# 331658260/Drone-YOLO

Hardware: AMD Instinct MI355X
Metric: images/sec @640x640 Drone-YOLO-s (higher is better)
Workload: dtype fp16; 1 GPU; Drone-YOLO-s (yolov8s-p2-repvgg.yaml, nc=10) inference 640x640: layout+forward+decode+NMS, inputs resident in HBM; fp16 storage / fp32 accumulate (BASELINE config 2 names bf16: bf16 storage fails the IoU >= 0.999 bar - 0.995 - so the headline runs the 16-bit format that meets it; same MFMA rate, same bytes); batch_per_gpu=256, global_batch=256, parallelism=batch-split x1, no collective, hipgraph=True, streams=2, max_det=300

## Files before the change

drone-yolo_amd/csrc/layout_ops.hip:

```cpp
#include "common_hip.h"

namespace dy {

template <typename T>
__global__ __launch_bounds__(256) void nchw_to_nhwc_kernel(const float* __restrict__ src, T* __restrict__ dst, int n,
                                                           int c, int hw, int c_pad, int ld) {
  constexpr int EPC = Elem<T>::EPC;
  const long long total = (long long)n * hw;
  for (long long pix = (long long)blockIdx.x * 256 + threadIdx.x; pix < total; pix += (long long)gridDim.x * 256) {
    const int img = (int)(pix / hw);
    const int p = (int)(pix - (long long)img * hw);
    const float* s = src + (size_t)img * c * hw + p;
    T* d = dst + (size_t)pix * ld;
    for (int c0 = 0; c0 < c_pad; c0 += EPC) {
      float f[EPC];
#pragma unroll
      for (int e = 0; e < EPC; ++e) f[e] = (c0 + e < c) ? s[(size_t)(c0 + e) * hw] : 0.f;
      *reinterpret_cast<u32x4*>(d + c0) = Chunk<T>::pack(f);
    }
  }
}

__global__ __launch_bounds__(256) void nchw_to_nhwc_split_kernel(const float* __restrict__ src, unsigned char* __restrict__ dst, int n, int c, int hw, int c_pad, int ld) {
  const long long total = (long long)n * hw;
// ... 100 lines not shown
  u32x4* tmp = cur + tot;
  const int img = blockIdx.x / cgroups;
  const int cg = blockIdx.x - img * cgroups;
  const size_t base = (size_t)img * hw * ld + (size_t)cg * G * EPC;
  for (int i = threadIdx.x; i < tot; i += 512) {
    const int p = i / G, g = i - p * G;
    cur[i] = *reinterpret_cast<const u32x4*>(x + base + (size_t)p * ld + g * EPC);
  }
  __syncthreads();
  T* outs[3] = {y1, y2, y3};
#pragma unroll 1
  for (int pass = 0; pass < 3; ++pass) {
    for (int i = threadIdx.x; i < tot; i += 512) {
      const int p = i / G, g = i - p * G;
      const int yy = p / w, xx = p - yy * w;
      const int x0 = xx - r < 0 ? 0 : xx - r, x1 = xx + r >= w ? w - 1 : xx + r;
      u32x4 m = cur[(yy * w + x0) * G + g];
      for (int q = x0 + 1; q <= x1; ++q) m = chunk_max<T>(m, cur[(yy * w + q) * G + g]);
      tmp[i] = m;
    }
    __syncthreads();
    T* o = outs[pass];
    for (int i = threadIdx.x; i < tot; i += 512) {
      const int p = i / G, g = i - p * G;
      const int yy = p / w, xx = p - yy * w;
      const int y0 = yy - r < 0 ? 0 : yy - r, y1e = yy + r >= h ? h - 1 : yy + r;
      u32x4 m = tmp[(y0 * w + xx) * G + g];
      for (int q = y0 + 1; q <= y1e; ++q) m = chunk_max<T>(m, tmp[(q * w + xx) * G + g]);
      cur[i] = m;
      *reinterpret_cast<u32x4*>(o + base + (size_t)p * ld + g * EPC) = m;
    }
    __syncthreads();
  }
}

struct ChunkPair {
  u32x4 hi, lo;
};
__device__ __forceinline__ ChunkPair pair_max(const ChunkPair a, const ChunkPair b) {
  float fa[8], fb[8];
  join8(a.hi, a.lo, fa);
  join8(b.hi, b.lo, fb);
  const f16x8 ah = __builtin_bit_cast(f16x8, a.hi), al = __builtin_bit_cast(f16x8, a.lo), bh = __builtin_bit_cast(f16x8, b.hi), bl = __builtin_bit_cast(f16x8, b.lo);
  f16x8 h, l;
#pragma unroll
  for (int e = 0; e < 8; ++e) {
    const bool tb = fb[e] > fa[e];
    h[e] = tb ? bh[e] : ah[e];
    l[e] = tb ? bl[e] : al[e];
  }
  return ChunkPair{__builtin_bit_cast(u32x4, h), __builtin_bit_cast(u32x4, l)};
}

__global__ __launch_bounds__(512) void sppf_maxpool3_split_kernel(const unsigned char* __restrict__ x, unsigned char* __restrict__ y1, unsigned char* __restrict__ y2,
                                                                  unsigned char* __restrict__ y3, int h, int w, int cgroups, int G, int ld, int r) {
  extern __shared__ __attribute__((aligned(16))) unsigned char dyn_smem[];
  const int hw = h * w, tot = hw * G;
  ChunkPair* cur = reinterpret_cast<ChunkPair*>(dyn_smem);
  ChunkPair* tmp = cur + tot;
  const int img = blockIdx.x / cgroups;
  const int cg = blockIdx.x - img * cgroups;
  const size_t base = ((size_t)img * hw * ld + (size_t)cg * G * 8) * 4;
  for (int i = threadIdx.x; i < tot; i += 512) {
    const int p = i / G, g = i - p * G;
    const unsigned char* s = x + base + ((size_t)p * ld + g * 8) * 4;
    cur[i] = ChunkPair{*reinterpret_cast<const u32x4*>(s), *reinterpret_cast<const u32x4*>(s + 16)};
// ... 230 lines not shown
  const int epc = 16 / es;
  DY_REQUIRE(n > 0 && h > 0 && w > 0 && c > 0 && c % epc == 0 && ld >= c && ld % epc == 0, DY_ERR_INVALID_ARG,
             "dy_sppf_maxpool3: c/ld must be multiples of %d", epc);
  DY_REQUIRE(k >= 1 && (k & 1), DY_ERR_INVALID_ARG, "dy_sppf_maxpool3: k must be odd");
  DY_REQUIRE(aligned16(x) && aligned16(y1) && aligned16(y2) && aligned16(y3), DY_ERR_INVALID_ARG,
             "dy_sppf_maxpool3: views must be 16-byte aligned");
  DY_REQUIRE((long long)h * w <= 4608, DY_ERR_UNSUPPORTED, "dy_sppf_maxpool3: h*w=%d exceeds the LDS-resident limit 4608", h * w);
  hipStream_t st = reinterpret_cast<hipStream_t>(stream);
  const int cchunks = c / epc;
  int G = 1;
  for (int g = 8; g >= 1; --g)
    if (cchunks % g == 0 && (size_t)h * w * 32 * g <= 147456) {
      G = g;
      break;
    }
  const size_t smem = (size_t)h * w * 32 * G;
  const int cgroups = cchunks / G;
  if (dtype == DY_F16X2) {
    DY_REQUIRE(c % 8 == 0, DY_ERR_INVALID_ARG, "dy_sppf_maxpool3: DY_F16X2 needs c in groups of 8 channels");
    const int pairs = c / 8;
    int Gp = 1;
    for (int g = 4; g >= 1; --g)
      if (pairs % g == 0 && (size_t)h * w * 64 * g <= 147456) {
        Gp = g;
        break;
      }
    const size_t sm = (size_t)h * w * 64 * Gp;
    DY_REQUIRE(sm <= 147456, DY_ERR_UNSUPPORTED, "dy_sppf_maxpool3: DY_F16X2 map of %d pixels exceeds the LDS-resident limit", h * w);
    if (sm > 48 * 1024) (void)hipFuncSetAttribute((const void*)sppf_maxpool3_split_kernel, hipFuncAttributeMaxDynamicSharedMemorySize, (int)sm);
    hipLaunchKernelGGL(sppf_maxpool3_split_kernel, dim3((unsigned)(n * (pairs / Gp))), dim3(512), sm, st, (const unsigned char*)x, (unsigned char*)y1, (unsigned char*)y2,
                       (unsigned char*)y3, h, w, pairs / Gp, Gp, ld, k / 2);
    return check_launch("sppf_maxpool3_split_kernel");
  }
  const dim3 grid((unsigned)(n * cgroups));
#define DY_SPPF_LAUNCH(T)                                                                                          \
  do {                                                                                                              \
    if (smem > 48 * 1024)                                                                                           \
      (void)hipFuncSetAttribute((const void*)sppf_maxpool3_kernel<T>, hipFuncAttributeMaxDynamicSharedMemorySize,  \
                                (int)smem);                                                                         \
    hipLaunchKernelGGL((sppf_maxpool3_kernel<T>), grid, dim3(512), smem, st, (const T*)x, (T*)y1, (T*)y2, (T*)y3, h, \
                       w, cgroups, G, ld, k / 2);                                                                   \
  } while (0)
  if (dtype == DY_BF16)
    DY_SPPF_LAUNCH(bf16_t);
  else if (dtype == DY_F16)
    DY_SPPF_LAUNCH(f16_t);
  else if (dtype == DY_FP8)
    DY_SPPF_LAUNCH(fp8_t);
  else
    DY_SPPF_LAUNCH(float);
#undef DY_SPPF_LAUNCH
  return check_launch("sppf_maxpool3_kernel");
}

extern "C" int32_t dy_quantize_fp8_nhwc(const void* src, void* dst, int64_t rows, int32_t c, int32_t ld_src, int32_t ld_dst, int32_t src_dtype, float act_scale,
                                        dy_stream_t stream) {
  const int es = dtype_size_no_fp8(src_dtype);
  DY_REQUIRE(src && dst && es && rows > 0 && c > 0 && act_scale > 0.f, DY_ERR_INVALID_ARG, "dy_quantize_fp8_nhwc: bad arguments");
  DY_REQUIRE(c % 16 == 0 && ld_src >= c && ld_dst >= c && (ld_src * es) % 16 == 0 && ld_dst % 16 == 0 && aligned16(src) && aligned16(dst), DY_ERR_INVALID_ARG,
             "dy_quantize_fp8_nhwc: c must be a multiple of 16 and both views whole 16-byte chunks");
  hipStream_t st = reinterpret_cast<hipStream_t>(stream);
  const int grid = grid_for((long long)rows * (c / 16));
  const float inv = 1.f / act_scale;
  if (src_dtype == DY_BF16)
    hipLaunchKernelGGL((quantize_fp8_kernel<bf16_t>), dim3(grid), dim3(256), 0, st, (const bf16_t*)src, (fp8_t*)dst, (long long)rows, c / 16, ld_src, ld_dst, inv);
  else if (src_dtype == DY_F16)
    hipLaunchKernelGGL((quantize_fp8_kernel<f16_t>), dim3(grid), dim3(256), 0, st, (const f16_t*)src, (fp8_t*)dst, (long long)rows, c / 16, ld_src, ld_dst, inv);
  else
// ... 85 lines not shown
```

drone-yolo_amd/_lib.py:

```python
from __future__ import annotations

import ctypes as C
import os

_HERE = os.path.dirname(os.path.abspath(__file__))
LIB_PATH = os.path.join(_HERE, "lib", "libdyolo.so")

DY_BF16, DY_F16, DY_F32, DY_FP8, DY_F16X2 = 0, 1, 2, 3, 4
DY_ACT_NONE, DY_ACT_SILU, DY_ACT_SILU_L2E = 0, 1, 2
DY_MAX_LEVELS = 8
DY_WLAYOUT_ROWS, DY_WLAYOUT_HALO3X3, DY_WLAYOUT_FRAG1X1 = 0, 1, 2

_vp, _i32, _f32, _i64 = C.c_void_p, C.c_int32, C.c_float, C.c_int64


class PackJob(C.Structure):
    _fields_ = [("w", C.c_void_p), ("s_co", C.c_int64), ("s_ci", C.c_int64), ("s_r", C.c_int64), ("s_q", C.c_int64),
                ("cout", C.c_int32), ("cin", C.c_int32), ("ksize", C.c_int32), ("transpose_flip", C.c_int32), ("cin_logical", C.c_int32),
                ("w_layout", C.c_int32), ("dst", C.c_void_p), ("dst_elems", C.c_int64)]


class ConvDesc(C.Structure):

    _fields_ = [
# ... 92 lines not shown
        ("fuse_score", _i32), ("max_time_lost", _i32),
    ]


class LossDesc(C.Structure):

    _fields_ = [
        ("level", _vp * DY_MAX_LEVELS),
        ("h", _i32 * DY_MAX_LEVELS), ("w", _i32 * DY_MAX_LEVELS), ("ld", _i32 * DY_MAX_LEVELS),
        ("stride", _f32 * DY_MAX_LEVELS),
        ("n_levels", _i32), ("batch", _i32), ("nc", _i32), ("reg_max", _i32),
        ("gt", _vp), ("gmax", _i32), ("topk", _i32),
        ("alpha", _f32), ("beta", _f32), ("box_gain", _f32), ("cls_gain", _f32), ("dfl_gain", _f32),
        ("out", _vp), ("out_owner", _vp), ("workspace", _vp), ("workspace_bytes", _i64),
        ("grad_level", _vp * DY_MAX_LEVELS), ("ld_grad", _i32 * DY_MAX_LEVELS),
    ]


class C2fTailDesc(C.Structure):

    _fields_ = [
        ("t", _vp), ("buf", _vp), ("y", _vp), ("w3", _vp), ("b3", _vp), ("w1", _vp), ("b1", _vp),
        ("batch", _i32), ("h", _i32), ("w", _i32), ("hidden", _i32), ("cout", _i32), ("n_bottlenecks", _i32), ("shortcut", _i32),
        ("ld_t", _i32), ("ld_buf", _i32), ("ld_y", _i32), ("dtype", _i32), ("act_l2e", _i32),
    ]


class C2fFrontDesc(C.Structure):

    _fields_ = [
        ("x", _vp), ("other", _vp), ("y", _vp), ("w3", _vp), ("b3", _vp), ("w1", _vp), ("b1", _vp),
        ("batch", _i32), ("h", _i32), ("w", _i32), ("cin", _i32), ("cmid", _i32), ("c_other", _i32), ("cout", _i32),
        ("ld_x", _i32), ("ld_other", _i32), ("ld_y", _i32), ("act", _i32), ("dtype", _i32),
    ]


class C2fDesc(C.Structure):

    _fields_ = [
        ("x", _vp), ("x_lo", _vp), ("y", _vp), ("w_cv1", _vp), ("w_m_cv1", _vp), ("w_m_cv2", _vp), ("w_cv2", _vp), ("bias", _vp),
        ("batch", _i32), ("h", _i32), ("w", _i32), ("cin", _i32), ("cin_lo", _i32), ("hidden", _i32), ("cout", _i32),
        ("ld_x", _i32), ("ld_x_lo", _i32), ("ld_y", _i32), ("shortcut", _i32), ("dtype", _i32), ("act_l2e", _i32),
    ]


class Stem2Desc(C.Structure):

    _fields_ = [
        ("x", _vp), ("w0", _vp), ("b0", _vp), ("w1", _vp), ("b1", _vp), ("y", _vp),
        ("n", _i32), ("h", _i32), ("w", _i32), ("ld_y", _i32), ("act0", _i32), ("act1", _i32), ("dtype", _i32),
        ("w1_scale", _vp),
    ]


class BnDesc(C.Structure):

    _fields_ = [
        ("z", _vp), ("y", _vp), ("addend", _vp), ("dy", _vp), ("dz", _vp),
        ("rows", _i64),
        ("c", _i32), ("ld_z", _i32), ("ld_y", _i32), ("ld_add", _i32), ("ld_dy", _i32), ("ld_dz", _i32), ("dtype", _i32), ("act", _i32),
        ("gamma", _vp), ("beta", _vp), ("mean", _vp), ("rstd", _vp), ("running_mean", _vp), ("running_var", _vp),
        ("eps", _f32), ("momentum", _f32),
        ("dgamma", _vp), ("dbeta", _vp), ("workspace", _vp), ("workspace_bytes", _i64), ("partial_slabs", _i32),
    ]


DY_AUG_FLIPLR, DY_AUG_FLIPUD, DY_AUG_HSV_OFF = 1, 2, 4


class AugSrc(C.Structure):

    _fields_ = [("index", _i32), ("x1a", _i32), ("y1a", _i32), ("x2a", _i32), ("y2a", _i32), ("x1b", _i32), ("y1b", _i32), ("reserved", _i32)]


class AugRow(C.Structure):

    _fields_ = [("n_src", _i32), ("ch", _i32), ("cw", _i32), ("flags", _i32), ("src", AugSrc * 4), ("minv", _f32 * 9), ("hsv", _f32 * 3)]


SIGNATURES = {
    "dy_version": (_i32, []),
    "dy_last_error_string": (C.c_char_p, []),
    "dy_last_kernel_name": (C.c_char_p, []),
    "dy_dtype_size": (_i32, [_i32]),
    "dy_pack_conv_weights_table_bytes": (C.c_int64, [_i32]),
    "dy_pack_conv_weights_table": (_i32, [C.POINTER(PackJob), _i32, _i32, _vp, C.c_int64, C.POINTER(C.c_int32)]),
    "dy_pack_conv_weights_batched": (_i32, [_vp, _i32, _i32, _i32, _vp]),
    "dy_conv_k_pad": (_i32, [_i32, _i32, _i32]),
    "dy_conv_cout_pad": (_i32, [_i32]),
    "dy_conv2d_nhwc": (_i32, [C.POINTER(ConvDesc), _vp]),
    "dy_conv_stats_written": (_i32, []),
    "dy_c2f_fused_supported": (_i32, [_i32, _i32, _i32, _i32, _i32, _i32]),
    "dy_c2f_fused": (_i32, [C.POINTER(C2fDesc), _vp]),
    "dy_c2f_tail_fused_supported": (_i32, [_i32, _i32, _i32, _i32, _i32, _i32, _i32]),
    "dy_c2f_tail_fused": (_i32, [C.POINTER(C2fTailDesc), _vp]),
    "dy_c2f_front_fused_supported": (_i32, [_i32, _i32, _i32, _i32, _i32, _i32, _i32, _i32, _i32]),
    "dy_c2f_front_fused": (_i32, [C.POINTER(C2fFrontDesc), _vp]),
    "dy_stem2_fused_supported": (_i32, [_i32, _i32, _i32, _i32, _i32, _i32]),
    "dy_stem2_fused": (_i32, [C.POINTER(Stem2Desc), _vp]),
    "dy_stem_conv3x3s2_nchw": (_i32, [_vp, _vp, _vp, _vp, _i32, _i32, _i32, _i32, _i32, _i32, _i32, _i32, _vp]),
    "dy_stem_conv3x3s2_nchw_u8": (_i32, [_vp, _f32, _vp, _vp, _vp, _i32, _i32, _i32, _i32, _i32, _i32, _i32, _i32, _vp]),
    "dy_nchw_f32_to_nhwc": (_i32, [_vp, _vp, _i32, _i32, _i32, _i32, _i32, _i32, _i32, _vp]),
    "dy_resize_bilinear_u8_nchw_f32": (_i32, [_vp, _vp, _i32, _i32, _i32, _i32, _i32, _i32, _vp]),
    "dy_scale_img_nchw_f32": (_i32, [_vp, _vp, _i32, _i32, _i32, _i32, _i32, _i32, _i32, _i32, _i32, _f32, _vp]),
    "dy_nhwc_to_nchw_f32": (_i32, [_vp, _vp, _i32, _i32, _i32, _i32, _i32, _i32, _vp]),
    "dy_upsample2x_nhwc": (_i32, [_vp, _vp, _i32, _i32, _i32, _i32, _i32, _i32, _i32, _vp]),
    "dy_copy_nhwc": (_i32, [_vp, _vp, _i32, _i32, _i32, _i32, _i32, _i32, _i32, _vp]),
    "dy_sppf_maxpool3": (_i32, [_vp, _vp, _vp, _vp, _i32, _i32, _i32, _i32, _i32, _i32, _i32, _vp]),
    "dy_detect_decode": (_i32, [C.POINTER(DecodeDesc), _vp]),
    "dy_detect_head_decode_supported": (_i32, [_i32, _i32, _i32, _i32, _i32]),
    "dy_detect_head_decode": (_i32, [C.POINTER(HeadDecodeDesc), _vp]),
    "dy_nms_workspace_bytes": (_i64, [_i32, _i32]),
    "dy_nms": (_i32, [C.POINTER(NmsDesc), _vp]),
    "dy_nms_small_cap": (_i32, []),
    "dy_scale_boxes": (_i32, [_vp, _vp, _vp, _i32, _i32, _vp]),
    "dy_val_match": (_i32, [C.POINTER(ValMatchDesc), _vp]),
    "dy_track_state_bytes": (_i64, [_i32, _i32]),
    "dy_track_workspace_bytes": (_i64, [_i32, _i32, _i32]),
    "dy_track_reset": (_i32, [_vp, _i32, _i32, _vp]),
    "dy_track_step": (_i32, [C.POINTER(TrackDesc), _vp]),
    "dy_detection_loss_workspace_bytes": (_i64, [_i32, _i32, _i32, _i32]),
    "dy_conv2d_wgrad_nhwc": (_i32, [C.POINTER(ConvDesc), _vp, _i32, _vp, _vp]),
    "dy_conv2d_wgrad_nhwc_ws": (_i32, [C.POINTER(ConvDesc), _vp, _i32, _vp, _vp, C.c_int64, _vp]),
    "dy_conv2d_wgrad_workspace_bytes": (C.c_int64, [C.POINTER(ConvDesc), _i32]),
    "dy_quantize_fp8_nhwc": (_i32, [_vp, _vp, _i64, _i32, _i32, _i32, _i32, _f32, _vp]),
    "dy_pack_conv_weights": (_i32, [_vp, _i64, _i64, _i64, _i64, _i32, _i32, _i32, _i32, _i32, _vp, _i64, _i32, _i32, _vp]),
    "dy_detect_branch_fused_supported": (_i32, [_i32, _i32, _i32, _i32, _i32, _i32, _i32]),
    "dy_detect_branch_fused": (_i32, [C.POINTER(BranchDesc), _vp]),
    "dy_nms_reset_counts": (_i32, [_vp, _i32, _vp]),
    "dy_conv2d_grouped_bwd_nhwc": (_i32, [C.POINTER(ConvDesc), _vp, _i32, _vp, _vp, _vp, _i32, _vp, _i32, _vp]),
# ... 58 lines not shown
```

drone-yolo_amd/hip_ops.py:

```python
from __future__ import annotations

import contextlib
import ctypes as C
from typing import List, NamedTuple, Optional, Sequence, Tuple

import os
import warnings

import torch

from . import _lib
from ._lib import DY_ACT_NONE, DY_ACT_SILU, DY_ACT_SILU_L2E, BnDesc, BranchDesc, C2fDesc, C2fFrontDesc, C2fTailDesc, ConvDesc, DecodeDesc, HeadDecodeDesc, LossDesc, NmsDesc, Stem2Desc, TileMergeDesc, TrackDesc, ValMatchDesc, check, lib

FP8 = torch.float8_e4m3fn
F16X2 = torch.complex32
_DTYPES = {torch.bfloat16: _lib.DY_BF16, torch.float16: _lib.DY_F16, torch.float32: _lib.DY_F32, FP8: _lib.DY_FP8, F16X2: _lib.DY_F16X2}
warnings.filterwarnings("ignore", message="ComplexHalf support is experimental")

_FP8 = {"act_scale": 1.0}


def set_fp8_act_scale(scale: float) -> None:
    if not scale > 0:
        raise ValueError("fp8 activation scale must be positive")
    _FP8["act_scale"] = float(scale)


def fp8_act_scale() -> float:
    return _FP8["act_scale"]


_absmax_log: Optional[list] = None


class observe_absmax:

    def __enter__(self):
        global _absmax_log
        _absmax_log = []
        return _absmax_log

    def __exit__(self, *exc):
        global _absmax_log
        _absmax_log = None
        return False
# ... 1518 lines not shown
            raise ValueError("PackedC2fFront: the stride-2 convolution did not pack as DY_WLAYOUT_HALO3X3")
        self.w3, self.b3 = p3.w, p3.b
        self.w1, self.b1 = pack_frag1x1(w1, b1, dtype, device)
        self.act, self.dtype = int(act), dtype


def c2f_front_fused_supported(cin: int, cmid: int, c_other: int, cout: int, dtype: torch.dtype, act: int = DY_ACT_SILU, k: int = 3, stride: int = 2, groups: int = 1) -> bool:
    return dtype in (torch.bfloat16, torch.float16) and bool(lib().dy_c2f_front_fused_supported(cin, cmid, c_other, cout, k, stride, groups, int(act), dy_dtype(dtype)))


def c2f_front_fused(x: torch.Tensor, pk: PackedC2fFront, other: Optional[torch.Tensor] = None, out: Optional[torch.Tensor] = None) -> torch.Tensor:
    require_device(x, "c2f front input")
    n, c, h, w = x.shape
    ho, wo = conv_out_hw(h, w, 3, 2, 1)
    if x.dtype != pk.dtype or c != pk.cin or (other is None) != (pk.c_other == 0):
        raise ValueError("c2f_front_fused: inputs do not match the packed pair")
    if other is not None:
        require_device(other, "c2f front second source")
        if tuple(other.shape) != (n, pk.c_other, ho, wo) or other.dtype != pk.dtype:
            raise ValueError("c2f_front_fused: other must be a (N, c_other, Ho, Wo) view of the input's dtype")
    if out is None:
        out = alloc_nhwc(n, pk.cout, ho, wo, x.dtype, x.device)
    elif tuple(out.shape) != (n, pk.cout, ho, wo) or out.dtype != x.dtype:
        raise ValueError("c2f_front_fused: out must be a (N, cout, Ho, Wo) view of the input's dtype")
    d = C2fFrontDesc()
    (d.x, d.ld_x), (d.y, d.ld_y) = view_params(x), view_params(out)
    if other is not None:
        d.other, d.ld_other = view_params(other)
    d.w3, d.b3, d.w1, d.b1 = pk.w3.data_ptr(), pk.b3.data_ptr(), pk.w1.data_ptr(), pk.b1.data_ptr()
    d.batch, d.h, d.w, d.cin, d.cmid, d.c_other, d.cout = n, h, w, pk.cin, pk.cmid, pk.c_other, pk.cout
    d.act, d.dtype = pk.act, dy_dtype(x.dtype)
    _launch(lib().dy_c2f_front_fused, (C.byref(d),), keep=(d, x, other, out, pk))
    return out
```

drone-yolo_amd/nn/modules/block.py:

```python
from __future__ import annotations

import torch
import torch.nn as nn

from ... import hip_ops as H
from .conv import Conv, _PackedMixin, _train_forward, fold_conv_bn

__all__ = ("DFL", "SPPF", "C2f", "Bottleneck", "RepVGGBlock", "SEBlock", "conv_bn")


class DFL(nn.Module):

    def __init__(self, c1=16):
        super().__init__()
        self.conv = nn.Conv2d(c1, 1, 1, bias=False).requires_grad_(False)
        self.conv.weight.data[:] = torch.arange(c1, dtype=torch.float).view(1, c1, 1, 1)
        self.c1 = c1

    def forward(self, x):
        raise RuntimeError("DFL is fused into Detect's decode kernel (dy_detect_decode); call Detect instead")


class Bottleneck(nn.Module):

# ... 118 lines not shown
                m(ybuf[:, (1 + i) * c : (2 + i) * c], out=ybuf[:, (2 + i) * c : (3 + i) * c])
            t = self.m[-1].cv1(ybuf[:, nm * c :])
            return H.c2f_tail_fused(t, ybuf, self._packed_tail(x.dtype, x.device), out=out)
        ybuf = H.alloc_nhwc(n, (2 + len(self.m)) * c, h, w, x.dtype, x.device)
        self._cv1(x, ybuf[:, : 2 * c], front, kw)
        for i, m in enumerate(self.m):
            m(ybuf[:, (1 + i) * c : (2 + i) * c], out=ybuf[:, (2 + i) * c : (3 + i) * c])
        return self.cv2(ybuf, out=out)


def _c2f_fp8_internal(self, x, out=None):
    n, _, h, w = x.shape
    c = self.c
    ybuf = H.alloc_nhwc(n, (2 + len(self.m)) * c, h, w, H.FP8, x.device)
    self.cv1(x, out=ybuf[:, : 2 * c], out_dtype=H.FP8)
    for i, m in enumerate(self.m):
        m(ybuf[:, (1 + i) * c : (2 + i) * c], out=ybuf[:, (2 + i) * c : (3 + i) * c])
    return self.cv2(ybuf, out=out, out_dtype=x.dtype)


C2f._forward_fp8_internal = _c2f_fp8_internal


class SPPF(nn.Module):

    def __init__(self, c1, c2, k=5):
        super().__init__()
        c_ = c1 // 2
        self.cv1 = Conv(c1, c_, 1, 1)
        self.cv2 = Conv(c_ * 4, c2, 1, 1)
        self.k = k
        self.m = nn.MaxPool2d(kernel_size=k, stride=1, padding=k // 2)

    def forward(self, x, out=None):
        if self.training:
            return _train_forward(self, "sppf_train", x, out=out)
        n, _, h, w = x.shape
        c_ = self.cv1.conv.out_channels
        ybuf = H.alloc_nhwc(n, 4 * c_, h, w, x.dtype, x.device)
        self.cv1(x, out=ybuf[:, :c_])
        H.sppf_maxpool3(ybuf[:, :c_], ybuf[:, c_ : 2 * c_], ybuf[:, 2 * c_ : 3 * c_], ybuf[:, 3 * c_ :], self.k)
        return self.cv2(ybuf, out=out)


def conv_bn(in_channels, out_channels, kernel_size, stride, padding, groups=1):
    result = nn.Sequential()
    result.add_module("conv", nn.Conv2d(in_channels, out_channels, kernel_size, stride, padding, groups=groups, bias=False))
    result.add_module("bn", nn.BatchNorm2d(out_channels))
    return result


class SEBlock(nn.Module):

    def __init__(self, input_channels, internal_neurons):
        super().__init__()
        self.down = nn.Conv2d(input_channels, internal_neurons, kernel_size=1, stride=1, bias=True)
        self.up = nn.Conv2d(internal_neurons, input_channels, kernel_size=1, stride=1, bias=True)
        self.input_channels = input_channels

    def forward(self, inputs):
        raise NotImplementedError("SEBlock (RepVGGBlock use_se=True) has no HIP kernel: not on the Drone-YOLO path")


class RepVGGBlock(_PackedMixin, nn.Module):

    def __init__(self, in_channels, out_channels, kernel_size=3, stride=1, padding=1, dilation=1, groups=1,
                 padding_mode="zeros", deploy=False, use_se=False):
        super().__init__()
        if dilation != 1 or padding_mode != "zeros" or kernel_size != 3:
            raise NotImplementedError("RepVGGBlock is built for 3x3, dilation 1, zero padding")
        self.deploy = deploy
        self.groups = groups
        self.in_channels = in_channels
        self.stride, self.padding = stride, padding
# ... 62 lines not shown
```

include/dyolo.h:

```cpp
#ifndef DYOLO_H_
#define DYOLO_H_

#include <stdint.h>

#ifdef __cplusplus
extern "C" {
#endif

#define DYOLO_VERSION_MAJOR 0
#define DYOLO_VERSION_MINOR 1

typedef void* dy_stream_t;

typedef enum dy_status {
  DY_OK = 0,
  DY_ERR_INVALID_ARG = -1,
  DY_ERR_UNSUPPORTED = -2,
  DY_ERR_LAUNCH = -3,
  DY_ERR_WORKSPACE = -4
} dy_status;

typedef enum dy_dtype { DY_BF16 = 0, DY_F16 = 1, DY_F32 = 2, DY_FP8 = 3, DY_F16X2 = 4 } dy_dtype;
typedef enum dy_act { DY_ACT_NONE = 0, DY_ACT_SILU = 1, DY_ACT_SILU_L2E = 2 } dy_act;
typedef enum dy_wlayout { DY_WLAYOUT_ROWS = 0, DY_WLAYOUT_HALO3X3 = 1, DY_WLAYOUT_FRAG1X1 = 2 } dy_wlayout;
// ... 83 lines not shown
  const float* bias;
  int32_t batch, h, w, cin, cin_lo, hidden, cout, ld_x, ld_x_lo, ld_y, shortcut, dtype;
  int32_t act_l2e;
} dy_c2f_desc;
int32_t dy_c2f_fused_supported(int32_t cin, int32_t cin_lo, int32_t hidden, int32_t cout, int32_t n_bottlenecks, int32_t dtype);
int32_t dy_c2f_fused(const dy_c2f_desc* d, dy_stream_t stream);

typedef struct dy_c2f_tail_desc {
  const void* t;
  const void* buf;
  void* y;
  const void* w3;
  const float* b3;
  const void* w1;
  const float* b1;
  int32_t batch, h, w, hidden, cout, n_bottlenecks, shortcut, ld_t, ld_buf, ld_y, dtype;
  int32_t act_l2e;
} dy_c2f_tail_desc;
int32_t dy_c2f_tail_fused_supported(int32_t hidden, int32_t cout, int32_t n_bottlenecks, int32_t ksize1, int32_t ksize2, int32_t groups, int32_t dtype);
int32_t dy_c2f_tail_fused(const dy_c2f_tail_desc* d, dy_stream_t stream);

typedef struct dy_c2f_front_desc {
  const void* x;
  const void* other;
  void* y;
  const void* w3;
  const float* b3;
  const void* w1;
  const float* b1;
  int32_t batch, h, w, cin, cmid, c_other, cout, ld_x, ld_other, ld_y, act, dtype;
} dy_c2f_front_desc;
int32_t dy_c2f_front_fused_supported(int32_t cin, int32_t cmid, int32_t c_other, int32_t cout, int32_t ksize, int32_t stride, int32_t groups, int32_t act, int32_t dtype);
int32_t dy_c2f_front_fused(const dy_c2f_front_desc* d, dy_stream_t stream);

int32_t dy_stem_conv3x3s2_nchw(const float* x, const void* w, const float* bias, void* y, int32_t n, int32_t cin,
                               int32_t h, int32_t w_in, int32_t cout, int32_t ld_y, int32_t act, int32_t dtype,
                               dy_stream_t stream);

int32_t dy_stem_conv3x3s2_nchw_u8(const uint8_t* x, float divisor, const void* w, const float* bias, void* y, int32_t n, int32_t cin,
                                  int32_t h, int32_t w_in, int32_t cout, int32_t ld_y, int32_t act, int32_t dtype, dy_stream_t stream);

typedef struct dy_stem2_desc {
  const float* x;
  const void* w0;
  const float* b0;
  const void* w1;
  const float* b1;
  void* y;
  int32_t n, h, w, ld_y, act0, act1, dtype;
  const float* w1_scale;
} dy_stem2_desc;
int32_t dy_stem2_fused_supported(int32_t cin, int32_t c0, int32_t c1, int32_t h, int32_t w, int32_t dtype);
int32_t dy_stem2_fused(const dy_stem2_desc* d, dy_stream_t stream);

int32_t dy_letterbox_u8_to_nchw_f32(const uint8_t* src, float* dst, int32_t n, int32_t h0, int32_t w0, int32_t new_w, int32_t new_h,
                                    int32_t top, int32_t left, int32_t hn, int32_t wn, int32_t swap_rb, float pad_value,
                                    dy_stream_t stream);

int32_t dy_resize_bilinear_u8_nchw_f32(const uint8_t* src, float* dst, int32_t n, int32_t c, int32_t h, int32_t w, int32_t ho, int32_t wo, dy_stream_t stream);
int32_t dy_scale_img_nchw_f32(const float* src, float* dst, int32_t n, int32_t c, int32_t h, int32_t w, int32_t hs, int32_t ws, int32_t ho, int32_t wo,
                              int32_t flip_lr, float pad, dy_stream_t stream);

int32_t dy_tiles_u8_to_nchw_f32(const uint8_t* frame, const int32_t* offsets_yx, float* dst, int32_t k, int32_t hf, int32_t wf, int32_t th,
                                int32_t tw, int32_t swap_rb, float pad_value, dy_stream_t stream);
int32_t dy_rows_to_pred(const float* rows, const int32_t* counts, const int32_t* offsets_yx, float* pred, int32_t k, int32_t max_det,
                        int32_t nc, dy_stream_t stream);
// ... 227 lines not shown
```

Measured before the change: 21210 images/sec.

## Add persistent register-blocked SPPF 5x5 maxpool kernel with prefetch and packed max

Adds a specialized SPPF kernel for k=5 in f16/bf16. It is persistent over image/channel-group tiles and prefetches the next tile's input into registers while the current tile runs three cascaded pools. Each thread computes R output rows, sharing vertical partial maxima across them, and uses packed v_pk_max instructions. bf16 values are remapped to an integer-comparable key so integer max can be used. SPPF is a small part of the network, so the whole-model effect is likely limited, and the bf16 key path and buffer-rsrc bounds add complexity.

```diff
diff --git a/drone-yolo_amd/csrc/layout_ops.hip b/drone-yolo_amd/csrc/layout_ops.hip
--- a/drone-yolo_amd/csrc/layout_ops.hip
+++ b/drone-yolo_amd/csrc/layout_ops.hip
@@ -156,6 +156,142 @@
     }
     __syncthreads();
   }
+}
+
+template <typename T>
+__device__ __forceinline__ u32x4 pool_max(u32x4 a, u32x4 b);
+template <typename T>
+__device__ __forceinline__ u32x4 pool_key(u32x4 v) {
+  return v;
+}
+template <>
+__device__ __forceinline__ u32x4 pool_key<bf16_t>(u32x4 v) {
+  typedef __attribute__((ext_vector_type(8))) short s16x8;
+  const s16x8 k = __builtin_bit_cast(s16x8, v);
+  return __builtin_bit_cast(u32x4, (s16x8)(k ^ ((k >> 15) & (short)0x7fff)));
+}
+template <>
+__device__ __forceinline__ u32x4 pool_max<bf16_t>(u32x4 a, u32x4 b) {
+  u32x4 r;
+#pragma unroll
+  for (int e = 0; e < 4; ++e) {
+    unsigned o;
+    asm("v_pk_max_i16 %0, %1, %2" : "=v"(o) : "v"(a[e]), "v"(b[e]));
+    r[e] = o;
+  }
+  return r;
+}
+template <>
+__device__ __forceinline__ u32x4 pool_max<f16_t>(u32x4 a, u32x4 b) {
+  u32x4 r;
+#pragma unroll
+  for (int e = 0; e < 4; ++e) {
+    unsigned o;
+    asm("v_pk_max_f16 %0, %1, %2" : "=v"(o) : "v"(a[e]), "v"(b[e]));
+    r[e] = o;
+  }
+  return r;
+}
+
+constexpr int kPoolThreads = 512;
+#ifndef DY_SPPF_WGS_PER_CU
+#define DY_SPPF_WGS_PER_CU 2
+#endif
+
+template <typename T, int R>
+__global__ __launch_bounds__(kPoolThreads) __attribute__((amdgpu_waves_per_eu(4, 4))) void sppf_pool5_kernel(const T* __restrict__ x, T* __restrict__ y1, T* __restrict__ y2,
+                                                                                                             T* __restrict__ y3, int h, int w, int cgroups, int G, int ld,
+                                                                                                             int ygroups, int ntiles) {
+  extern __shared__ __attribute__((aligned(16))) unsigned char dyn_smem[];
+  constexpr int EPC = Elem<T>::EPC;
+  const int tid = threadIdx.x, wG = w * G;
+  const int yg = tid / wG, rem = tid - yg * wG;
+  const int xx = rem / G, g = rem - xx * G;
+  const bool live = yg < ygroups;
+  const int r0 = live ? yg * R : 0;
+  const int nvalid = live ? (h - r0 < R ? h - r0 : R) : 0;
+  const unsigned rowB = (unsigned)wG * 16u;
+  const unsigned a0 = (unsigned)(r0 * wG + rem) * 16u;
+  int dx[4];
+  {
+    const int q[4] = {xx - 2, xx - 1, xx + 1, xx + 2};
+#pragma unroll
+    for (int i = 0; i < 4; ++i) dx[i] = ((q[i] < 0 ? 0 : (q[i] >= w ? w - 1 : q[i])) - xx) * G * 16;
+  }
+  unsigned ca[R + 4];
+#pragma unroll
+  for (int i = 0; i < R + 4; ++i) {
+    const int row = r0 - 2 + i;
+    ca[i] = (unsigned)((row < 0 ? 0 : (row >= h ? h - 1 : row)) * wG + rem) * 16u;
+  }
+  constexpr unsigned kOob = 0xfffffc00u, kWindow = 0x80000000u;
+  unsigned goffB = (unsigned)(((size_t)(r0 * w + xx) * ld + (size_t)g * EPC) * sizeof(T));
+  const unsigned gstepB = (unsigned)((size_t)w * ld * sizeof(T));
+  auto tile_rsrc = [&](const T* ptr, int tile) -> __amdgpu_buffer_rsrc_t {
+    const int img = tile / cgroups, cg = tile - img * cgroups;
+    return __builtin_amdgcn_make_buffer_rsrc(const_cast<T*>(ptr + (size_t)img * h * w * ld + (size_t)cg * G * EPC), 0, kWindow, 0x00020000);
+  };
+  auto voff = [&](int j) -> unsigned { return j < nvalid ? goffB + (unsigned)j * gstepB : kOob; };
+#define DY_POOL_PIN_ROW0() asm volatile("" : "+v"(goffB))
+  auto lds = [&](unsigned addr) -> u32x4& { return *reinterpret_cast<u32x4*>(dyn_smem + addr); };
+
+  u32x4 pre[R];
+  auto fetch = [&](int tile) {
+    const __amdgpu_buffer_rsrc_t xr = tile_rsrc(x, tile);
+    DY_POOL_PIN_ROW0();
+#pragma unroll
+    for (int j = 0; j < R; ++j) pre[j] = __builtin_amdgcn_raw_buffer_load_b128(xr, voff(j), 0, 0);
+  };
+  int tile = blockIdx.x;
+  fetch(tile);
+#pragma unroll
+  for (int j = 0; j < R; ++j)
+    if (j < nvalid) lds(a0 + j * rowB) = pool_key<T>(pre[j]);
+  __syncthreads();
+  for (; tile < ntiles; tile += gridDim.x) {
+    const int next = tile + gridDim.x;
+    if (next < ntiles) fetch(next);
+#pragma unroll
+    for (int pass = 0; pass < 3; ++pass) {
+      const __amdgpu_buffer_rsrc_t yr = tile_rsrc(pass == 0 ? y1 : (pass == 1 ? y2 : y3), tile);
+      u32x4 res[R];
+      asm volatile("" : "+v"(dx[0]), "+v"(dx[1]), "+v"(dx[2]), "+v"(dx[3]));
+      {
+        u32x4 t[R + 3];
+        u32x4 vprev;
+#pragma unroll
+        for (int i = 0; i < R + 4; ++i) {
+          const unsigned a = ca[i];
+          const u32x4 l2 = lds(a + dx[0]), l1 = lds(a + dx[1]), c = lds(a), r1 = lds(a + dx[2]), r2 = lds(a + dx[3]);
+          const u32x4 v = pool_max<T>(pool_max<T>(pool_max<T>(pool_max<T>(l2, l1), c), r1), r2);
+          if (i > 0) t[i - 1] = pool_max<T>(vprev, v);
+          if (i >= 4) res[i - 4] = pool_max<T>(pool_max<T>(t[i - 4], t[i - 2]), v);
+          vprev = v;
+          __builtin_amdgcn_sched_barrier(0);
+        }
+      }
+      __syncthreads();
+      if (pass < 2 || next < ntiles) {
+#pragma unroll
+        for (int j = 0; j < R; ++j)
+          if (j < nvalid) lds(a0 + j * rowB) = pass < 2 ? res[j] : pool_key<T>(pre[j]);
+      }
+      DY_POOL_PIN_ROW0();
+#pragma unroll
+      for (int j = 0; j < R; ++j) __builtin_amdgcn_raw_buffer_store_b128(pool_key<T>(res[j]), yr, voff(j), 0, 0);
+      __syncthreads();
+    }
+  }
+}
+
+#undef DY_POOL_PIN_ROW0
+
+static inline int pool5_rows_per_thread(int h, int w, int G, int ld, int es) {
+  if ((long long)h * w * ld * es >= (1ll << 31)) return 0;
+  const int cands[2] = {4, 7};
+  for (int R : cands)
+    if ((long long)((h + R - 1) / R) * w * G <= kPoolThreads) return R;
+  return 0;
 }
 
 struct ChunkPair {
@@ -452,8 +588,37 @@
                        (unsigned char*)y3, h, w, pairs / Gp, Gp, ld, k / 2);
     return check_launch("sppf_maxpool3_split_kernel");
   }
+  if (k == 5 && (dtype == DY_F16 || dtype == DY_BF16)) {
+    const int R = pool5_rows_per_thread(h, w, G, ld, es);
+    if (R) {
+      const int ygroups = (h + R - 1) / R, ntiles = n * cgroups;
+      const size_t sm = (size_t)h * w * G * 16;
+      static const int wgs = [] {
+        int dev = 0, cus = 0;
+        if (hipGetDevice(&dev) != hipSuccess || hipDeviceGetAttribute(&cus, hipDeviceAttributeMultiprocessorCount, dev) != hipSuccess || cus <= 0) cus = 256;
+        return DY_SPPF_WGS_PER_CU * cus;
+      }();
+      const dim3 pgrid((unsigned)(ntiles < wgs ? ntiles : wgs));
+#define DY_POOL5_LAUNCH(T, RR)                                                                                                                            \
+  do {                                                                                                                                                    \
+    if (sm > 48 * 1024) (void)hipFuncSetAttribute((const void*)sppf_pool5_kernel<T, RR>, hipFuncAttributeMaxDynamicSharedMemorySize, (int)sm);            \
+    hipLaunchKernelGGL((sppf_pool5_kernel<T, RR>), pgrid, dim3(kPoolThreads), sm, st, (const T*)x, (T*)y1, (T*)y2, (T*)y3, h, w, cgroups, G, ld, ygroups, \
+                       ntiles);                                                                                                                           \
+  } while (0)
+      if (dtype == DY_F16 && R == 4)
+        DY_POOL5_LAUNCH(f16_t, 4);
+      else if (dtype == DY_F16)
+        DY_POOL5_LAUNCH(f16_t, 7);
+      else if (R == 4)
+        DY_POOL5_LAUNCH(bf16_t, 4);
+      else
+        DY_POOL5_LAUNCH(bf16_t, 7);
+#undef DY_POOL5_LAUNCH
+      return check_launch("sppf_pool5_kernel");
+    }
+  }
   const dim3 grid((unsigned)(n * cgroups));
-#define DY_SPPF_LAUNCH(T)                                                                                          \
+#define DY_SPPF_LAUNCH(T)                                                                                         \
   do {                                                                                                              \
     if (smem > 48 * 1024)                                                                                           \
       (void)hipFuncSetAttribute((const void*)sppf_maxpool3_kernel<T>, hipFuncAttributeMaxDynamicSharedMemorySize,  \
```

Result: no change. 21320 images/sec, median of 6 (+0.5%).

## Fuse SPPF cv1 1x1 conv with the three cascaded maxpools in one kernel

Applied to the files above, without the earlier changes.

Adds a HIP kernel that computes the SPPF cv1 1x1 convolution with MFMA for one image and one 64-channel slice. It keeps the SiLU output in LDS and runs the three cascaded separable max-pool passes there, writing all four concat slices directly. This removes a kernel launch and the global-memory round trip of the cv1 output between the conv and maxpool kernels. The trade-off is one block per image and slice at a small 20x20 map, which can limit occupancy and tiling efficiency compared with the generic conv path. The Python SPPF module falls back to the old path when the shape is unsupported.

```diff
diff --git a/drone-yolo_amd/_lib.py b/drone-yolo_amd/_lib.py
--- a/drone-yolo_amd/_lib.py
+++ b/drone-yolo_amd/_lib.py
@@ -148,6 +148,15 @@
         ("x", _vp), ("other", _vp), ("y", _vp), ("w3", _vp), ("b3", _vp), ("w1", _vp), ("b1", _vp),
         ("batch", _i32), ("h", _i32), ("w", _i32), ("cin", _i32), ("cmid", _i32), ("c_other", _i32), ("cout", _i32),
         ("ld_x", _i32), ("ld_other", _i32), ("ld_y", _i32), ("act", _i32), ("dtype", _i32),
+    ]
+
+
+class SppfFrontDesc(C.Structure):
+
+    _fields_ = [
+        ("x", _vp), ("y", _vp), ("w1", _vp), ("b1", _vp),
+        ("batch", _i32), ("h", _i32), ("w", _i32), ("cin", _i32), ("cmid", _i32), ("k", _i32),
+        ("ld_x", _i32), ("ld_y", _i32), ("act", _i32), ("dtype", _i32), ("bias_last", _i32),
     ]
 
 
@@ -212,6 +221,8 @@
     "dy_c2f_tail_fused": (_i32, [C.POINTER(C2fTailDesc), _vp]),
     "dy_c2f_front_fused_supported": (_i32, [_i32, _i32, _i32, _i32, _i32, _i32, _i32, _i32, _i32]),
     "dy_c2f_front_fused": (_i32, [C.POINTER(C2fFrontDesc), _vp]),
+    "dy_sppf_front_fused_supported": (_i32, [_i32, _i32, _i32, _i32, _i32, _i32]),
+    "dy_sppf_front_fused": (_i32, [C.POINTER(SppfFrontDesc), _vp]),
     "dy_stem2_fused_supported": (_i32, [_i32, _i32, _i32, _i32, _i32, _i32]),
     "dy_stem2_fused": (_i32, [C.POINTER(Stem2Desc), _vp]),
     "dy_stem_conv3x3s2_nchw": (_i32, [_vp, _vp, _vp, _vp, _i32, _i32, _i32, _i32, _i32, _i32, _i32, _i32, _vp]),
diff --git a/drone-yolo_amd/csrc/sppf_front.hip b/drone-yolo_amd/csrc/sppf_front.hip
--- /dev/null
+++ b/drone-yolo_amd/csrc/sppf_front.hip
@@ -0,0 +1,272 @@
+#include "common_hip.h"
+
+namespace DY_NS {
+
+constexpr int kSfThreads = 512;
+constexpr int kSfMaxPix = 512;
+constexpr int kSfWBytes = 64 * 128;
+constexpr int kSfMaxPieces = (kSfMaxPix / 8 + 8 + 7) / 8;
+
+struct SppfFrontArgs {
+  const void* x;
+  const void* w;
+  const float* bias;
+  void* y;
+  int H, W, HW, PR;
+  int Cin, Kpad, ldx, ldy, Cmid, nslices, nblk, r;
+  int dy64, dx64;
+  unsigned xbytes, wbytes;
+};
+
+typedef __attribute__((ext_vector_type(8))) short s16x8;
+typedef __attribute__((ext_vector_type(4))) short s16x4;
+
+__device__ __forceinline__ u32x4 sf_key(u32x4 v) {
+  const u32x4 m = __builtin_bit_cast(u32x4, __builtin_bit_cast(s16x8, v) >> (short)15);
+  return v ^ (m & 0x7fff7fffu);
+}
+__device__ __forceinline__ u32x2 sf_key(u32x2 v) {
+  const u32x2 m = __builtin_bit_cast(u32x2, __builtin_bit_cast(s16x4, v) >> (short)15);
+  return v ^ (m & 0x7fff7fffu);
+}
+__device__ __forceinline__ u32x4 sf_max(u32x4 a, u32x4 b) {
+  return __builtin_bit_cast(u32x4, __builtin_elementwise_max(__builtin_bit_cast(s16x8, a), __builtin_bit_cast(s16x8, b)));
+}
+
+template <typename T>
+__device__ __forceinline__ u32x2 sf_round4(const float (&v)[4]) {
+  if constexpr (sizeof(T) == 2 && __is_same(T, f16_t)) {
+    typedef __attribute__((ext_vector_type(2))) float f32x2;
+    typedef __attribute__((ext_vector_type(2))) _Float16 f16x2v;
+    const f16x2v lo = __builtin_convertvector(f32x2{v[0], v[1]}, f16x2v), hi = __builtin_convertvector(f32x2{v[2], v[3]}, f16x2v);
+    return u32x2{__builtin_bit_cast(unsigned, lo), __builtin_bit_cast(unsigned, hi)};
+  } else {
+    typedef __attribute__((ext_vector_type(4))) T t4;
+    t4 o;
+#pragma unroll
+    for (int e = 0; e < 4; ++e) o[e] = Elem<T>::from_f32(v[e]);
+    return __builtin_bit_cast(u32x2, o);
+  }
+}
+
+template <int R, typename At>
+__device__ __forceinline__ u32x4 sf_window(const At& at, unsigned char* base, int q, int step, int lo, int hi) {
+  if constexpr (R > 0) {
+    u32x4 v[2 * R + 1];
+#pragma unroll
+    for (int t = -R; t <= R; ++t) {
+      const int d = t < -lo ? -lo : (t > hi ? hi : t);
+      v[t + R] = *at(base, q + d * step);
+    }
+    u32x4 m = v[0];
+#pragma unroll
+    for (int t = 1; t <= 2 * R; ++t) m = sf_max(m, v[t]);
+    return m;
+  } else {
+    u32x4 m = *at(base, q - lo * step);
+    for (int d = 1 - lo; d <= hi; ++d) m = sf_max(m, *at(base, q + d * step));
+    return m;
+  }
+}
+
+template <typename T, bool BIAS_LAST, int R>
+__global__ __launch_bounds__(kSfThreads) void sppf_front_fused_kernel(const SppfFrontArgs p) {
+  static_assert(sizeof(T) == 2, "16-bit storage");
+  extern __shared__ __attribute__((aligned(1024))) unsigned char dyn_smem[];
+
+  const int tid = threadIdx.x, lane = tid & 63;
+  const int wave = __builtin_amdgcn_readfirstlane(tid >> 6);
+  const int lq = lane >> 4, lr = lane & 15;
+  const unsigned L = xcd_remap(blockIdx.x, (unsigned)p.nblk);
+  const int img = (int)(L / (unsigned)p.nslices), sl = (int)(L - (unsigned)img * (unsigned)p.nslices);
+  const int A_BYTES = p.PR * 128, STAGE = A_BYTES + kSfWBytes;
+  const int npa = p.PR >> 3, npieces = npa + 8;
+  const int nfrag = p.PR >> 4;
+
+  constexpr unsigned kOob = 0xfffffff0u;
+  const T* ximg = reinterpret_cast<const T*>(p.x) + (size_t)img * (size_t)p.HW * (size_t)p.ldx;
+  const __amdgpu_buffer_rsrc_t xrs = __builtin_amdgcn_make_buffer_rsrc(const_cast<T*>(ximg), 0, p.xbytes, 0x00020000);
+  const __amdgpu_buffer_rsrc_t wrs = __builtin_amdgcn_make_buffer_rsrc(const_cast<void*>(p.w), 0, p.wbytes, 0x00020000);
+  const int prow = lane >> 3;
+  unsigned voff[kSfMaxPieces];
+#pragma unroll
+  for (int i = 0; i < kSfMaxPieces; ++i) {
+    const int pi = wave + 8 * i;
+    const int row = (pi < npa ? pi : pi - npa) * 8 + prow;
+    const unsigned sw = (unsigned)(((lane & 7) ^ ((row >> 1) & 7)) * 16);
+    if (pi < npa) voff[i] = row < p.HW ? (unsigned)(row * p.ldx) * 2u + sw : kOob;
+    else voff[i] = (unsigned)((sl * 64 + row) * p.Kpad) * 2u + sw;
+  }
+  auto issue = [&](int step, int stage) {
+    unsigned char* sbase = dyn_smem + stage * STAGE;
+    const unsigned soff = (unsigned)step * 128u;
+#pragma unroll
+    for (int i = 0; i < kSfMaxPieces; ++i) {
+      const int pi = wave + 8 * i;
+      if (pi < npa)
+        __builtin_amdgcn_raw_ptr_buffer_load_lds(xrs, (__attribute__((address_space(3))) void*)(sbase + pi * 1024), 16, (int)voff[i], (int)soff, 0, 0);
+      else if (pi < npieces)
+        __builtin_amdgcn_raw_ptr_buffer_load_lds(wrs, (__attribute__((address_space(3))) void*)(sbase + pi * 1024), 16, (int)voff[i], (int)soff, 0, 0);
+    }
+  };
+
+  f32x4 acc[4][4];
+  f32x4 bb[4];
+#pragma unroll
+  for (int j = 0; j < 4; ++j) {
+    bb[j] = *reinterpret_cast<const f32x4*>(p.bias + sl * 64 + j * 16 + lq * 4);
+#pragma unroll
+    for (int i = 0; i < 4; ++i) acc[i][j] = BIAS_LAST ? f32x4{0.f, 0.f, 0.f, 0.f} : bb[j];
+  }
+
+  const int swz = lr >> 1;
+  auto compute = [&](int stage) {
+    const unsigned char* sa = dyn_smem + stage * STAGE + lr * 128;
+    const unsigned char* sb = sa + A_BYTES;
+#pragma unroll
+    for (int s = 0; s < 2; ++s) {
+      const int slot = ((s * 4 + lq) ^ swz) * 16;
+      u32x4 b[4];
+#pragma unroll
+      for (int j = 0; j < 4; ++j) b[j] = *reinterpret_cast<const u32x4*>(sb + j * 16 * 128 + slot);
+#pragma unroll
+      for (int i = 0; i < 4; ++i) {
+        const int f = wave + 8 * i;
+        if (f < nfrag) {
+          const u32x4 a = *reinterpret_cast<const u32x4*>(sa + f * 16 * 128 + slot);
+#pragma unroll
+          for (int j = 0; j < 4; ++j) acc[i][j] = Elem<T>::mma(b[j], a, acc[i][j]);
+        }
+      }
+    }
+  };
+
+  const int nsteps = p.Cin >> 6;
+  issue(0, 0);
+  for (int s = 0; s < nsteps; ++s) {
+    asm volatile("s_waitcnt vmcnt(0)" ::: "memory");
+    __syncthreads();
+    if (s + 1 < nsteps) issue(s + 1, (s + 1) & 1);
+    compute(s & 1);
+  }
+  __syncthreads();
+
+  unsigned char* const image = dyn_smem;
+  unsigned char* const temp = dyn_smem + A_BYTES;
+#pragma unroll
+  for (int i = 0; i < 4; ++i) {
+    const int f = wave + 8 * i;
+    if (f < nfrag) {
+      const int px = f * 16 + lr;
+#pragma unroll
+      for (int j = 0; j < 4; ++j) {
+        float v[4];
+#pragma unroll
+        for (int e = 0; e < 4; ++e) v[e] = silu_f32(BIAS_LAST ? acc[i][j][e] + bb[j][e] : acc[i][j][e]);
+        const u32x2 o = sf_round4<T>(v);
+        const int c = j * 2 + (lq >> 1);
+        *reinterpret_cast<u32x2*>(image + px * 128 + (((c ^ (px >> 1)) & 7) << 4) + (lq & 1) * 8) = sf_key(o);
+      }
+    }
+  }
+  __syncthreads();
+
+  const int g = tid & 7;
+  const int p0 = tid >> 3;
+  const int y0 = p0 / p.W, x0 = p0 - y0 * p.W;
+  auto at = [&](unsigned char* base, int q) -> u32x4* { return reinterpret_cast<u32x4*>(base + q * 128 + (((g ^ (q >> 1)) & 7) << 4)); };
+  T* const yimg = reinterpret_cast<T*>(p.y) + (size_t)img * (size_t)p.HW * (size_t)p.ldy + (size_t)(sl * 64 + g * 8);
+  for (int q = p0; q < p.HW; q += 64) *reinterpret_cast<u32x4*>(yimg + q * p.ldy) = sf_key(*at(image, q));
+#pragma unroll 1
+  for (int pass = 1; pass <= 3; ++pass) {
+    for (int q = p0, xx = x0; q < p.HW; q += 64) {
+      const int lo = xx < p.r ? xx : p.r, hi = xx + p.r >= p.W ? p.W - 1 - xx : p.r;
+      *at(temp, q) = sf_window<R>(at, image, q, 1, lo, hi);
+      xx += p.dx64;
+      if (xx >= p.W) xx -= p.W;
+    }
+    __syncthreads();
+    T* const yo = yimg + pass * p.Cmid;
+    for (int q = p0, xx = x0, yy = y0; q < p.HW; q += 64) {
+      const int lo = yy < p.r ? yy : p.r, hi = yy + p.r >= p.H ? p.H - 1 - yy : p.r;
+      const u32x4 m = sf_window<R>(at, temp, q, p.W, lo, hi);
+      *at(image, q) = m;
+      *reinterpret_cast<u32x4*>(yo + q * p.ldy) = sf_key(m);
+      xx += p.dx64, yy += p.dy64;
+      if (xx >= p.W) xx -= p.W, ++yy;
+    }
+    __syncthreads();
+  }
+}
+
+template <typename T>
+static int launch_sppf_front(const SppfFrontArgs& a, bool bias_last, hipStream_t st) {
+  const size_t smem = 2 * ((size_t)a.PR * 128 + kSfWBytes);
+  const dim3 grid((unsigned)a.nblk), block(kSfThreads);
+#define DY_SF_LAUNCH(BL, RR)                                                                                                     \
+  do {                                                                                                                           \
+    if (smem > 48 * 1024)                                                                                                        \
+      (void)hipFuncSetAttribute((const void*)sppf_front_fused_kernel<T, BL, RR>, hipFuncAttributeMaxDynamicSharedMemorySize, (int)smem); \
+    hipLaunchKernelGGL((sppf_front_fused_kernel<T, BL, RR>), grid, block, smem, st, a);                                          \
+  } while (0)
+  if (bias_last) {
+    if (a.r == 2) DY_SF_LAUNCH(true, 2);
+    else DY_SF_LAUNCH(true, 0);
+  } else {
+    if (a.r == 2) DY_SF_LAUNCH(false, 2);
+    else DY_SF_LAUNCH(false, 0);
+  }
+#undef DY_SF_LAUNCH
+  return check_launch("sppf_front_fused_kernel");
+}
+
+}
+
+using namespace DY_NS;
+
+#ifndef DYOLO_L2E_BUILD
+extern "C" int32_t dy_sppf_front_fused_supported(int32_t cin, int32_t cmid, int32_t h, int32_t w, int32_t k, int32_t dtype) {
+  if (!(dtype == DY_BF16 || dtype == DY_F16)) return 0;
+  if (cin < 64 || cin % 64 || cmid < 64 || cmid % 64 || h < 1 || w < 1 || k < 1 || !(k & 1)) return 0;
+  if (cmid % 128 != 0 && cmid % 80 == 0) return 0;
+  return (long long)h * w <= kSfMaxPix;
+}
+
+namespace dy_l2e {
+int32_t sppf_front_entry(const dy_sppf_front_desc* d, dy_stream_t stream);
+}
+namespace dy {
+int32_t sppf_front_entry(const dy_sppf_front_desc* d, dy_stream_t stream);
+}
+extern "C" int32_t dy_sppf_front_fused(const dy_sppf_front_desc* d, dy_stream_t stream) {
+  return (d != nullptr && d->act == DY_ACT_SILU_L2E) ? dy_l2e::sppf_front_entry(d, stream) : dy::sppf_front_entry(d, stream);
+}
+#endif
+
+namespace DY_NS {
+int32_t sppf_front_entry(const dy_sppf_front_desc* d, dy_stream_t stream) {
+  DY_REQUIRE(d && d->x && d->y && d->w1 && d->b1, DY_ERR_INVALID_ARG, "dy_sppf_front_fused: null pointer");
+  DY_REQUIRE(d->act == DY_ACT_SILU || d->act == DY_ACT_SILU_L2E, DY_ERR_UNSUPPORTED, "dy_sppf_front_fused: cv1 must carry SiLU (act %d)", d->act);
+  DY_REQUIRE(dy_sppf_front_fused_supported(d->cin, d->cmid, d->h, d->w, d->k, d->dtype), DY_ERR_UNSUPPORTED,
+             "dy_sppf_front_fused: built for 16-bit storage, cin and c_ multiples of 64 (c_ not on the 160-wide tiles), odd k, h*w <= %d (got cin %d c_ %d map %dx%d k %d dtype %d): "
+             "run dy_conv2d_nhwc and dy_sppf_maxpool3", kSfMaxPix, d->cin, d->cmid, d->h, d->w, d->k, d->dtype);
+  DY_REQUIRE(d->batch > 0 && d->ld_x >= d->cin && d->ld_y >= 4 * d->cmid, DY_ERR_INVALID_ARG, "dy_sppf_front_fused: bad dims / pitches");
+  DY_REQUIRE(d->ld_x % 8 == 0 && d->ld_y % 8 == 0 && aligned16(d->x) && aligned16(d->y) && aligned16(d->w1) && aligned16(d->b1), DY_ERR_INVALID_ARG,
+             "dy_sppf_front_fused: views must be whole 16-byte chunks (16-byte stores)");
+  const int kpad = dy_conv_k_pad(d->cin, 1, d->dtype), cpad = dy_conv_cout_pad(d->cmid);
+  const long long hw = (long long)d->h * d->w;
+  DY_REQUIRE(kpad == d->cin && (long long)cpad * kpad * 2 < (1ll << 31) && hw * d->ld_x * 2 < (1ll << 31) && hw * d->ld_y * 2 < (1ll << 31) &&
+                 (long long)d->batch * (d->cmid / 64) < (1ll << 31),
+             DY_ERR_UNSUPPORTED, "dy_sppf_front_fused: an image's view or the weight image exceeds 2 GiB (32-bit offsets)");
+  SppfFrontArgs a{};
+  a.x = d->x, a.w = d->w1, a.bias = d->b1, a.y = d->y;
+  a.H = d->h, a.W = d->w, a.HW = (int)hw, a.PR = ((int)hw + 15) / 16 * 16;
+  a.Cin = d->cin, a.Kpad = kpad, a.ldx = d->ld_x, a.ldy = d->ld_y, a.Cmid = d->cmid;
+  a.nslices = d->cmid / 64, a.nblk = d->batch * a.nslices, a.r = d->k / 2;
+  a.dy64 = 64 / d->w, a.dx64 = 64 % d->w;
+  a.xbytes = (unsigned)(((hw - 1) * d->ld_x + d->cin) * 2), a.wbytes = (unsigned)((long long)cpad * kpad * 2);
+  hipStream_t st = reinterpret_cast<hipStream_t>(stream);
+  const bool bias_last = d->bias_last != 0;
+  return d->dtype == DY_BF16 ? launch_sppf_front<bf16_t>(a, bias_last, st) : launch_sppf_front<f16_t>(a, bias_last, st);
+}
+}
diff --git a/drone-yolo_amd/hip_ops.py b/drone-yolo_amd/hip_ops.py
--- a/drone-yolo_amd/hip_ops.py
+++ b/drone-yolo_amd/hip_ops.py
@@ -10,7 +10,7 @@
 import torch
 
 from . import _lib
-from ._lib import DY_ACT_NONE, DY_ACT_SILU, DY_ACT_SILU_L2E, BnDesc, BranchDesc, C2fDesc, C2fFrontDesc, C2fTailDesc, ConvDesc, DecodeDesc, HeadDecodeDesc, LossDesc, NmsDesc, Stem2Desc, TileMergeDesc, TrackDesc, ValMatchDesc, check, lib
+from ._lib import DY_ACT_NONE, DY_ACT_SILU, DY_ACT_SILU_L2E, BnDesc, BranchDesc, C2fDesc, C2fFrontDesc, C2fTailDesc, ConvDesc, DecodeDesc, HeadDecodeDesc, LossDesc, NmsDesc, SppfFrontDesc, Stem2Desc, TileMergeDesc, TrackDesc, ValMatchDesc, check, lib
 
 FP8 = torch.float8_e4m3fn
 F16X2 = torch.complex32
@@ -1595,3 +1595,44 @@
     d.act, d.dtype = pk.act, dy_dtype(x.dtype)
     _launch(lib().dy_c2f_front_fused, (C.byref(d),), keep=(d, x, other, out, pk))
     return out
+
+
+
+
+class PackedSppfFront:
+
+    def __init__(self, cv1, act: int, dtype: torch.dtype, device):
+        w1, b1 = cv1
+        self.cmid, self.cin = w1.shape[0], w1.shape[1]
+        if tuple(w1.shape[2:]) != (1, 1):
+            raise ValueError("PackedSppfFront: cv1 must be a 1x1 convolution")
+        self.act, self.dtype = int(act), dtype
+        own = conv_pack_plan(self.cmid, self.cin, 1, 1, 0, 1, self.act, dtype)
+        self.bias_last = own.layout == _lib.DY_WLAYOUT_FRAG1X1
+        pc = PackedConv(w1, b1, 1, 0, 1, self.act, dtype, device, halo=False)
+        if pc.layout != _lib.DY_WLAYOUT_ROWS:
+            raise ValueError("PackedSppfFront: cv1 did not pack as DY_WLAYOUT_ROWS")
+        self.w1, self.b1 = pc.w, pc.b
+
+
+def sppf_front_fused_supported(cin: int, cmid: int, h: int, w: int, k: int, dtype: torch.dtype, act: int = DY_ACT_SILU) -> bool:
+    return dtype in (torch.bfloat16, torch.float16) and int(act) in (DY_ACT_SILU, DY_ACT_SILU_L2E) and \
+        bool(lib().dy_sppf_front_fused_supported(cin, cmid, h, w, k, dy_dtype(dtype)))
+
+
+def sppf_front_fused(x: torch.Tensor, pk: PackedSppfFront, k: int, out: Optional[torch.Tensor] = None) -> torch.Tensor:
+    require_device(x, "sppf front input")
+    n, c, h, w = x.shape
+    if x.dtype != pk.dtype or c != pk.cin:
+        raise ValueError("sppf_front_fused: input does not match the packed cv1")
+    if out is None:
+        out = alloc_nhwc(n, 4 * pk.cmid, h, w, x.dtype, x.device)
+    elif tuple(out.shape) != (n, 4 * pk.cmid, h, w) or out.dtype != x.dtype:
+        raise ValueError("sppf_front_fused: out must be a (N, 4 * cmid, H, W) view of the input's dtype")
+    d = SppfFrontDesc()
+    (d.x, d.ld_x), (d.y, d.ld_y) = view_params(x), view_params(out)
+    d.w1, d.b1 = pk.w1.data_ptr(), pk.b1.data_ptr()
+    d.batch, d.h, d.w, d.cin, d.cmid, d.k = n, h, w, pk.cin, pk.cmid, int(k)
+    d.act, d.dtype, d.bias_last = pk.act, dy_dtype(x.dtype), int(pk.bias_last)
+    _launch(lib().dy_sppf_front_fused, (C.byref(d),), keep=(d, x, out, pk))
+    return out
diff --git a/drone-yolo_amd/nn/modules/block.py b/drone-yolo_amd/nn/modules/block.py
--- a/drone-yolo_amd/nn/modules/block.py
+++ b/drone-yolo_amd/nn/modules/block.py
@@ -174,14 +174,38 @@
         self.k = k
         self.m = nn.MaxPool2d(kernel_size=k, stride=1, padding=k // 2)
 
+    fuse_front = True
+
+    def _front_fusable(self, x) -> bool:
+        c = self.cv1.conv
+        if type(self.cv1) is not Conv or not isinstance(self.cv1.act, nn.SiLU) or c.kernel_size != (1, 1) or c.stride != (1, 1) or c.padding != (0, 0) or c.groups != 1:
+            return False
+        if x.shape[1] != c.in_channels:
+            return False
+        act = H.DY_ACT_SILU_L2E if H.scaled_domain() else H.DY_ACT_SILU
+        return H.sppf_front_fused_supported(c.in_channels, c.out_channels, x.shape[2], x.shape[3], self.k, x.dtype, act)
+
+    def _packed_front(self, dtype, device):
+        srcs = list(self.cv1.parameters()) + list(self.cv1.buffers())
+        key = (dtype, str(device), H.scaled_domain(), tuple((t.data_ptr(), t._version) for t in srcs))
+        cache = self.__dict__.get("_front_cache")
+        if cache is None or cache[0] != key:
+            w1, b1, act = self.cv1._folded()
+            cache = (key, H.PackedSppfFront((w1, b1), act, dtype, device))
+            self.__dict__["_front_cache"] = cache
+        return cache[1]
+
     def forward(self, x, out=None):
         if self.training:
             return _train_forward(self, "sppf_train", x, out=out)
         n, _, h, w = x.shape
         c_ = self.cv1.conv.out_channels
         ybuf = H.alloc_nhwc(n, 4 * c_, h, w, x.dtype, x.device)
-        self.cv1(x, out=ybuf[:, :c_])
-        H.sppf_maxpool3(ybuf[:, :c_], ybuf[:, c_ : 2 * c_], ybuf[:, 2 * c_ : 3 * c_], ybuf[:, 3 * c_ :], self.k)
+        if self.fuse_front and self._front_fusable(x):
+            H.sppf_front_fused(x, self._packed_front(x.dtype, x.device), self.k, out=ybuf)
+        else:
+            self.cv1(x, out=ybuf[:, :c_])
+            H.sppf_maxpool3(ybuf[:, :c_], ybuf[:, c_ : 2 * c_], ybuf[:, 2 * c_ : 3 * c_], ybuf[:, 3 * c_ :], self.k)
         return self.cv2(ybuf, out=out)
 
 
diff --git a/include/dyolo.h b/include/dyolo.h
--- a/include/dyolo.h
+++ b/include/dyolo.h
@@ -139,6 +139,16 @@
 } dy_c2f_front_desc;
 int32_t dy_c2f_front_fused_supported(int32_t cin, int32_t cmid, int32_t c_other, int32_t cout, int32_t ksize, int32_t stride, int32_t groups, int32_t act, int32_t dtype);
 int32_t dy_c2f_front_fused(const dy_c2f_front_desc* d, dy_stream_t stream);
+
+typedef struct dy_sppf_front_desc {
+  const void* x;
+  void* y;
+  const void* w1;
+  const float* b1;
+  int32_t batch, h, w, cin, cmid, k, ld_x, ld_y, act, dtype, bias_last;
+} dy_sppf_front_desc;
+int32_t dy_sppf_front_fused_supported(int32_t cin, int32_t cmid, int32_t h, int32_t w, int32_t k, int32_t dtype);
+int32_t dy_sppf_front_fused(const dy_sppf_front_desc* d, dy_stream_t stream);
 
 int32_t dy_stem_conv3x3s2_nchw(const float* x, const void* w, const float* bias, void* y, int32_t n, int32_t cin,
                                int32_t h, int32_t w_in, int32_t cout, int32_t ld_y, int32_t act, int32_t dtype,
```

New measurement: 20740 images/sec before, 20820 images/sec after, median of 6. About the same (+0.3%).
